# Ascend-Research/HeadPoseEstimation-WHENet

Measured on NVIDIA H100. Metric: head-crops/sec @224x224 bf16, higher is better.
Workload: dtype bf16

## Files before the change

### headposeestimation-whenet_b200/csrc/kernels_dwse.cuh

```cuda
#pragma once
#include <cuda.h>

#include "kernels_fused.cuh"

namespace whenet {
namespace fused {

struct alignas(64) DwSeParams {
    CUtensorMap tmE;
    CUtensorMap tmW;
    CUtensorMap tmX;
    CUtensorMap tmWx;
    const float* b_exp;
    const float* b_dw;
    int* tflag;
    void* out;
    float* partial;
    const float *w_se1t, *b_se1, *w_se2, *b_se2;
    float* gate;
    int Cse;
    float inv_hw;
    int se_tail;
    int scale_out;
    int C, pad;
    int n_chunks, chunks_per_cta;
    int N;
    int tiles_x, Ho_img;
};

template <int KS, int S, int HIN>
struct DwSeGeom {
    static constexpr int HO = (HIN + S - 1) / S;
    static constexpr int R = 7;
    static constexpr int SPR = HO / R;
    static constexpr int NSTRIPS = HO * SPR;
    static constexpr int PW = (HO - 1) * S + KS;
    static constexpr int NCOL = (R - 1) * S + KS;
};

template <int KS, int S, int HIN, int CC>
struct DwSeThreads { static constexpr int value = ((DwSeGeom<KS, S, HIN>::NSTRIPS * (CC / 4)) + 31) / 32 * 32; };

template <int KS, int S, int HIN, int CC>
constexpr size_t dwse_smem(int C, int Cse) {
    using G = DwSeGeom<KS, S, HIN>;
    return (size_t)2 * ((G::PW * G::PW * CC * 2 + 127) / 128 * 128)
           + (size_t)2 * ((CC * 4 + KS * KS * CC * 2 + 127) / 128 * 128)
           + (size_t)2 * G::NSTRIPS * CC * 4
           + (size_t)(C + Cse + 32) * 4 + 256;
}

template <typename T, int KS, int S, int HIN, int CC>
__device__ __forceinline__ void dw_strip(uint32_t erow, uint32_t cst, int cv, T* dst, int C, uint32_t red) {
    using G = DwSeGeom<KS, S, HIN>;
    constexpr int PITCH = CC * 2;
    const float4 bq = lds_f4(cst + (uint32_t)cv * 16);
    const uint32_t cst_h = cst + (uint32_t)(CC * 4 + cv * 8);
    __half2 hacc[G::R][2];
#pragma unroll
    for (int r = 0; r < G::R; ++r) { hacc[r][0] = __float2half2_rn(0.f); hacc[r][1] = __float2half2_rn(0.f); }
#pragma unroll
    for (int ky = 0; ky < KS; ++ky) {
        __half2 wr[KS][2];
#pragma unroll
        for (int kx = 0; kx < KS; ++kx) {
            uint32_t w0, w1;
            lds64(cst_h + (uint32_t)((ky * KS + kx) * CC) * 2, w0, w1);
            wr[kx][0] = *reinterpret_cast<__half2*>(&w0); wr[kx][1] = *reinterpret_cast<__half2*>(&w1);
        }
#pragma unroll
        for (int col = 0; col < G::NCOL; ++col) {
            uint32_t a, b;
            lds64(erow + (uint32_t)(col * PITCH), a, b);
            const __half2 x01 = *reinterpret_cast<__half2*>(&a), x23 = *reinterpret_cast<__half2*>(&b);
#pragma unroll
            for (int r = 0; r < G::R; ++r) {
                const int kx = col - r * S;
                if (kx >= 0 && kx < KS) {
                    hacc[r][0] = __hfma2(x01, wr[kx][0], hacc[r][0]);
                    hacc[r][1] = __hfma2(x23, wr[kx][1], hacc[r][1]);
                }
            }
        }
        erow += G::PW * PITCH;
    }
    const float2 sc = make_float2(kDwScale, kDwScale);
    float sum[4] = {0.f, 0.f, 0.f, 0.f};
#pragma unroll
    for (int r = 0; r < G::R; ++r) {
        float2 a0 = make_float2(bq.x, bq.y), a1 = make_float2(bq.z, bq.w);
        ffma2(a0, __half22float2(hacc[r][0]), sc);
        ffma2(a1, __half22float2(hacc[r][1]), sc);
        a0.x = swish_from_half(a0.x); a0.y = swish_from_half(a0.y);
        a1.x = swish_from_half(a1.x); a1.y = swish_from_half(a1.y);
        sum[0] += a0.x; sum[1] += a0.y; sum[2] += a1.x; sum[3] += a1.y;
        uint2 o;
        o.x = pack2<T>(a0.x, a0.y);
        o.y = pack2<T>(a1.x, a1.y);
        *reinterpret_cast<uint2*>(dst + (long long)r * C) = o;
    }
    asm volatile("st.shared.v4.f32 [%0], {%1,%2,%3,%4};" ::"r"(red), "f"(sum[0]), "f"(sum[1]), "f"(sum[2]), "f"(sum[3]) : "memory");
}

template <int NSTRIPS, int CC>
__device__ __forceinline__ void squeeze_sums(uint32_t red, float* dst, float* means, float inv_hw, int lane) {
    for (int cc = lane; cc < CC; cc += 32) {
        const uint32_t r0 = red + (uint32_t)(cc * 4);
        float s4[4] = {0.f, 0.f, 0.f, 0.f};
#pragma unroll
        for (int y = 0; y < NSTRIPS; ++y) {
            float t;
            asm volatile("ld.shared.f32 %0, [%1];" : "=f"(t) : "r"(r0 + (uint32_t)(y * CC * 4)));
            s4[y & 3] += t;
        }
        const float tot = (s4[0] + s4[1]) + (s4[2] + s4[3]);
        dst[cc] = tot;
        if (means) means[cc] = tot * inv_hw;
    }
}

template <typename T, int NT, int HO>
__device__ __forceinline__ void se_tail_gate(const DwSeParams& p, int n, T* out_n, float* sM) {
    const int C = p.C;
    se_gate_fc<NT>(sM, sM + C, p.w_se1t, p.b_se1, p.w_se2, p.b_se2, p.gate + (long long)n * C, C, p.Cse, sM);
    __syncthreads();
    if (p.scale_out) {
        const int cv8 = C >> 3, total = HO * HO * cv8;
        const float inv_cv8 = 1.0f / (float)cv8;
        for (int v = threadIdx.x; v < total; v += NT) {
            const int c8 = (v - div_small(v, inv_cv8) * cv8) * 8;
            uint4* ptr = reinterpret_cast<uint4*>(out_n) + v;
            *ptr = tc::scale8s<T>(__ldcg(ptr), tc::smem_u32(sM + c8));
        }
    }
}

template <typename T, int KS, int S, int HIN, int CC, bool SPATIAL = false>
__global__ void __launch_bounds__((DwSeThreads<KS, S, HIN, CC>::value)) dwse_kernel(const __grid_constant__ DwSeParams p) {
    using G = DwSeGeom<KS, S, HIN>;
    constexpr int NT = DwSeThreads<KS, S, HIN, CC>::value;
    constexpr int NW = NT / 32;
    constexpr int CV = CC / 4;
    constexpr int PITCH = CC * 2;
    constexpr int TILE_TX = G::PW * G::PW * PITCH;
    constexpr int TILE_BYTES = (TILE_TX + 127) / 128 * 128;
    constexpr int CST_TX = CC * 4 + KS * KS * CC * 2;
    constexpr int CST_BYTES = (CST_TX + 127) / 128 * 128;
    constexpr int RED_BYTES = G::NSTRIPS * CC * 4;
    extern __shared__ __align__(128) uint8_t smem_dw[];
    __shared__ __align__(8) uint64_t bars[4];
    __shared__ int s_abort_mem;
    volatile int* s_abort = &s_abort_mem;
    const uint32_t s0 = (tc::smem_u32(smem_dw) + 127u) & ~127u;
    const uint32_t sT = s0, sC = sT + 2 * TILE_BYTES, sR = sC + 2 * CST_BYTES;
    float* const sM = reinterpret_cast<float*>(smem_dw + (sR + 2 * RED_BYTES - tc::smem_u32(smem_dw)));
    const uint32_t b_full = tc::smem_u32(&bars[0]), b_empty = tc::smem_u32(&bars[2]);

    const int tid = threadIdx.x, warp = tid >> 5, lane = tid & 31;
    const int n = blockIdx.x;
    const int C = p.C;
    const int ch_begin = blockIdx.y * p.chunks_per_cta;
    const int ch_end = min(p.n_chunks, ch_begin + p.chunks_per_cta);
    const int Ho_img = SPATIAL ? p.Ho_img : G::HO;
    T* const out_n = reinterpret_cast<T*>(p.out) + (long long)n * Ho_img * Ho_img * C;

    if (tid == 0) {
        tc::mbar_init(&bars[0], 1); tc::mbar_init(&bars[1], 1);
        tc::mbar_init(&bars[2], NW); tc::mbar_init(&bars[3], NW);
        s_abort_mem = 0;
        asm volatile("fence.mbarrier_init.release.cluster;" ::: "memory");
        asm volatile("prefetch.tensormap [%0];" ::"l"(&p.tmE) : "memory");
        asm volatile("prefetch.tensormap [%0];" ::"l"(&p.tmW) : "memory");
    }
    __syncthreads();

    auto issue = [&](int ch, int buf) {
        const int cbase = SPATIAL ? 0 : ch * CC;
        const uint32_t bar = b_full + 8 * buf;
        tc::mbar::arrive_expect_tx(bar, (uint32_t)(TILE_TX + CST_TX));
        if (SPATIAL) {
            const int ty = ch / p.tiles_x, tx = ch - ty * p.tiles_x;
            tc::mbar::tma_4d(sT + buf * TILE_BYTES, &p.tmE, 0, tx * G::HO * S - p.pad, ty * G::HO * S - p.pad, n, bar);
        } else
            tc::mbar::tma_4d(sT + buf * TILE_BYTES, &p.tmE, cbase, -p.pad, -p.pad, n, bar);
        tc::mbar::tma_2d(sC + buf * CST_BYTES + CC * 4, &p.tmW, cbase, 0, bar);
        asm volatile("cp.async.bulk.shared::cluster.global.mbarrier::complete_tx::bytes [%0], [%1], %2, [%3];"
                     ::"r"(sC + buf * CST_BYTES), "l"(p.b_dw + cbase), "r"((uint32_t)(CC * 4)), "r"(bar) : "memory");
    };

    const int strip = tid / CV, cv = tid - strip * CV;
    const bool active = strip < G::NSTRIPS;
    const int oy = strip / G::SPR, ox0 = (strip - oy * G::SPR) * G::R;
    const uint32_t win = (uint32_t)(((oy * S) * G::PW + ox0 * S) * PITCH + cv * 8);

    if (tid == 0) {
        issue(ch_begin, 0);
        if (ch_begin + 1 < ch_end) issue(ch_begin + 1, 1);
    }

    for (int ch = ch_begin; ch < ch_end; ++ch) {
        const int it = ch - ch_begin, buf = it & 1;
        const uint32_t par = (uint32_t)(it >> 1) & 1u;
        tc::mbar::wait(b_full + 8 * buf, par, s_abort, p.tflag);
        if (active && !*s_abort) {
            T* dst;
            if (SPATIAL) {
                const int ty = ch / p.tiles_x, tx = ch - ty * p.tiles_x;
                dst = out_n + ((long long)(ty * G::HO + oy) * Ho_img + tx * G::HO + ox0) * C + cv * 4;
            } else
                dst = out_n + ((long long)oy * G::HO + ox0) * C + ch * CC + cv * 4;
            dw_strip<T, KS, S, HIN, CC>(sT + buf * TILE_BYTES + win, sC + buf * CST_BYTES, cv, dst, C,
                                        sR + (uint32_t)(buf * RED_BYTES + (strip * CC + cv * 4) * 4));
        }
        tc::mbar::arrive_warp(b_empty + 8 * buf);
        if (warp == 0) {
            tc::mbar::wait(b_empty + 8 * buf, par, s_abort, p.tflag);
            if (SPATIAL) squeeze_sums<G::NSTRIPS, CC>(sR + buf * RED_BYTES, p.partial + ((long long)n * p.n_chunks + ch) * C, nullptr, 0.f, lane);
            else squeeze_sums<G::NSTRIPS, CC>(sR + buf * RED_BYTES, p.partial + (long long)n * C + ch * CC, p.se_tail ? sM + ch * CC : nullptr, p.inv_hw, lane);
            __syncwarp();
            if (lane == 0 && ch + 2 < ch_end) issue(ch + 2, buf);
        }
    }
    __syncthreads();
    if (!SPATIAL && p.se_tail) se_tail_gate<T, NT, G::HO>(p, n, out_n, sM);
}

template <int KS, int S, int HIN, int CC, int CIN>
struct DwSeX {
    using G = DwSeGeom<KS, S, HIN>;
    static constexpr int NT = 256;
    static constexpr int NKB = (CIN + 63) / 64;
    static constexpr int KSTEPS = (CIN + 15) / 16;
    static constexpr int PIX = HIN * HIN;
    static constexpr int HALVES = (PIX + 63) / 64;
    static constexpr int XROWS = (PIX + 7) / 8 * 8;
    static_assert(HALVES == 4 || HALVES == 1, "14x14 or 7x7 maps");
    static constexpr int HPW = HALVES == 4 ? 2 : 1;
    static constexpr int NWG = HALVES == 4 ? CC : CC / 2;
    static_assert(NWG % 16 == 0 && NWG <= 128, "wgmma width");
    static_assert(G::NSTRIPS * (CC / 4) <= NT, "one depthwise strip per thread");
    static constexpr uint32_t X_KB = XROWS * 128, X_BYTES = NKB * X_KB;
    static constexpr uint32_t W_KB = CC * 128, W_BYTES = NKB * W_KB;
    static constexpr uint32_t TILE_BYTES = (G::PW * G::PW * CC * 2 + 127) / 128 * 128;
    static constexpr uint32_t CST_TX = CC * 4 + KS * KS * CC * 2;
    static constexpr uint32_t CST_BYTES = (CST_TX + 127) / 128 * 128;
    static constexpr uint32_t RED_BYTES = G::NSTRIPS * CC * 4;
    static constexpr uint32_t OFF_W = X_BYTES, OFF_T = OFF_W + 2 * W_BYTES, OFF_C = OFF_T + 2 * TILE_BYTES;
    static constexpr uint32_t OFF_R = OFF_C + 2 * CST_BYTES, OFF_M = OFF_R + 2 * RED_BYTES;
    static_assert((X_KB | W_KB | OFF_W | OFF_T) % 1024 == 0, "SWIZZLE_128B operands sit on 1024-byte boundaries");
    static constexpr size_t smem(int C, int Cse) { return (size_t)OFF_M + (size_t)(C + Cse + 32) * 4 + 1024; }
    static constexpr int CTAS_PER_SM = 2 * ((size_t)OFF_M + 4096 + 1024 + 1024) <= 228 * 1024 ? 2 : 1;
};

template <int KS, int S, int HIN, int CC, int CIN>
__global__ void __launch_bounds__(256, (DwSeX<KS, S, HIN, CC, CIN>::CTAS_PER_SM)) dwse_x_kernel(const __grid_constant__ DwSeParams p) {
    using X = DwSeX<KS, S, HIN, CC, CIN>;
    using G = typename X::G;
    using T = __nv_bfloat16;
    constexpr int NT = X::NT;
    constexpr int CV = CC / 4;
    extern __shared__ uint8_t smem_dwx[];
    __shared__ __align__(8) uint64_t bars[5];
    __shared__ int s_abort_mem;
    volatile int* s_abort = &s_abort_mem;
    const uint32_t s0 = (tc::smem_u32(smem_dwx) + 1023u) & ~1023u;
    const uint32_t sX = s0, sW = s0 + X::OFF_W, sT = s0 + X::OFF_T, sC = s0 + X::OFF_C, sR = s0 + X::OFF_R;
    float* const sM = reinterpret_cast<float*>(smem_dwx + (s0 + X::OFF_M - tc::smem_u32(smem_dwx)));
    const uint32_t b_x = tc::smem_u32(&bars[0]), b_w = b_x + 8, b_c = b_x + 24;

    const int tid = threadIdx.x, warp = tid >> 5, lane = tid & 31;
    const int wg = tid >> 7, wq = warp & 3;
    const int n = blockIdx.x;
    const int C = p.C, n_chunks = p.n_chunks;
    T* const out_n = reinterpret_cast<T*>(p.out) + (long long)n * G::HO * G::HO * C;

    if (tid == 0) {
        for (int i = 0; i < 5; ++i) tc::mbar_init(&bars[i], 1);
        s_abort_mem = 0;
        asm volatile("fence.mbarrier_init.release.cluster;" ::: "memory");
        asm volatile("prefetch.tensormap [%0];" ::"l"(&p.tmX) : "memory");
        asm volatile("prefetch.tensormap [%0];" ::"l"(&p.tmWx) : "memory");
        asm volatile("prefetch.tensormap [%0];" ::"l"(&p.tmW) : "memory");
    }
    for (uint32_t o = (uint32_t)tid * 16; o < 2 * X::TILE_BYTES; o += NT * 16) sts128(sT + o, make_uint4(0, 0, 0, 0));
    __syncthreads();

    auto issue_w = [&](int j) {
        const uint32_t bar = b_w + 8 * (j & 1);
        tc::mbar::arrive_expect_tx(bar, X::W_BYTES);
        for (int kb = 0; kb < X::NKB; ++kb) tc::mbar::tma_2d(sW + (j & 1) * X::W_BYTES + kb * X::W_KB, &p.tmWx, kb * 64, j * CC, bar);
    };
    auto issue_c = [&](int j) {
        const uint32_t bar = b_c + 8 * (j & 1), dst = sC + (j & 1) * X::CST_BYTES;
        tc::mbar::arrive_expect_tx(bar, X::CST_TX);
        tc::mbar::tma_2d(dst + CC * 4, &p.tmW, j * CC, 0, bar);
        asm volatile("cp.async.bulk.shared::cluster.global.mbarrier::complete_tx::bytes [%0], [%1], %2, [%3];"
                     ::"r"(dst), "l"(p.b_dw + j * CC), "r"((uint32_t)(CC * 4)), "r"(bar) : "memory");
    };
    if (tid == 0) {
        tc::mbar::arrive_expect_tx(b_x, X::X_BYTES);
        for (int kb = 0; kb < X::NKB; ++kb) tc::mbar::tma_2d(sX + kb * X::X_KB, &p.tmX, kb * 64, n * X::PIX, b_x);
        issue_w(0); issue_c(0);
        if (n_chunks > 1) { issue_w(1); issue_c(1); }
    }

    float acc[X::HPW][X::NWG / 2];
    auto mma = [&](int j) {
        tc::mbar::wait(b_x, 0, s_abort, p.tflag);
        tc::mbar::wait(b_w + 8 * (j & 1), (uint32_t)(j >> 1) & 1u, s_abort, p.tflag);
        const uint32_t wb = sW + (j & 1) * X::W_BYTES;
#pragma unroll
        for (int h = 0; h < X::HPW; ++h) {
            if constexpr (X::HALVES == 4) tc::wg_mma_m64<true, X::NWG>(acc[h], sX + (uint32_t)(wg * X::HPW + h) * 64 * 128, X::X_KB, wb, X::W_KB, X::KSTEPS);
            else tc::wg_mma_m64<true, X::NWG>(acc[h], sX, X::X_KB, wb + (uint32_t)wg * X::NWG * 128, X::W_KB, X::KSTEPS);
        }
    };
    auto epilogue = [&](int j) {
        const uint32_t tile = sT + (j & 1) * X::TILE_BYTES;
        const int c0 = X::HALVES == 4 ? 0 : wg * X::NWG;
        float2 bias[X::NWG / 8];
#pragma unroll
        for (int i = 0; i < X::NWG / 8; ++i) {
            const float* b = p.b_exp + j * CC + c0 + 8 * i + 2 * (lane & 3);
            bias[i] = make_float2(0.5f * __ldg(b), 0.5f * __ldg(b + 1));
        }
#pragma unroll
        for (int h = 0; h < X::HPW; ++h)
#pragma unroll
            for (int e = 0; e < 2; ++e) {
                const int pix = 64 * (X::HALVES == 4 ? wg * X::HPW + h : 0) + 16 * wq + (lane >> 2) + 8 * e;
                if (pix >= X::PIX) continue;
                const int y = pix / HIN, x = pix - y * HIN;
                const uint32_t prow = tile + (uint32_t)(((y + p.pad) * G::PW + x + p.pad) * CC + c0) * 2;
#pragma unroll
                for (int i = 0; i < X::NWG / 8; ++i) {
                    const int c = 8 * i + 2 * (lane & 3);
                    const float o0 = swish_from_half(fmaf(acc[h][4 * i + 2 * e], 0.5f, bias[i].x));
                    const float o1 = swish_from_half(fmaf(acc[h][4 * i + 2 * e + 1], 0.5f, bias[i].y));
                    asm volatile("st.shared.b32 [%0], %1;" ::"r"(prow + (uint32_t)c * 2), "r"(pack2<__half>(o0, o1)) : "memory");
                }
            }
    };

    const int strip = tid / CV, cv = tid - strip * CV;
    const bool active = strip < G::NSTRIPS;
    const int oy = strip / G::SPR, ox0 = (strip - oy * G::SPR) * G::R;
    const uint32_t win = (uint32_t)(((oy * S) * G::PW + ox0 * S) * CC * 2 + cv * 8);

    auto depthwise = [&](int j) {
        tc::mbar::wait(b_c + 8 * (j & 1), (uint32_t)(j >> 1) & 1u, s_abort, p.tflag);
        if (active && !*s_abort)
            dw_strip<T, KS, S, HIN, CC>(sT + (j & 1) * X::TILE_BYTES + win, sC + (j & 1) * X::CST_BYTES, cv,
                                        out_n + ((long long)oy * G::HO + ox0) * C + j * CC + cv * 4, C,
                                        sR + (uint32_t)((j & 1) * X::RED_BYTES + (strip * CC + cv * 4) * 4));
    };
    auto close = [&](int j) {
        if (warp == 0)
            squeeze_sums<G::NSTRIPS, CC>(sR + (j & 1) * X::RED_BYTES, p.partial + (long long)n * C + j * CC,
                                         p.se_tail ? sM + j * CC : nullptr, p.inv_hw, lane);
        if (tid == 0) {
            if (j + 3 < n_chunks) issue_w(j + 3);
            if (j + 2 < n_chunks) issue_c(j + 2);
        }
    };

    mma(0);
    tc::wg_wait<0>();
    epilogue(0);
    __syncthreads();
    if (tid == 0 && 2 < n_chunks) issue_w(2);
    for (int j = 0; j + 1 < n_chunks; ++j) {
        mma(j + 1);
        depthwise(j);
        tc::wg_wait<0>();
        epilogue(j + 1);
        __syncthreads();
        close(j);
    }
    depthwise(n_chunks - 1);
    __syncthreads();
    close(n_chunks - 1);
    __syncthreads();
    if (p.se_tail) se_tail_gate<T, NT, G::HO>(p, n, out_n, sM);
}

inline int dwse_chunk(int k, int s, int hin, int C) {
    if (hin == 14 && s == 1 && (k == 3 || k == 5) && C % 32 == 0) return 32;
    if (hin == 14 && s == 2 && k == 5 && C % 96 == 0) return 96;
    if (hin == 7 && s == 1 && (k == 3 || k == 5) && C % 128 == 0) return 128;
    return 0;
}

template <typename T>
int launch_dwse(cudaStream_t stream, DwSeParams p, int k, int s, int hin, int n_crops, int split) {
    const int CCr = dwse_chunk(k, s, hin, p.C);
    if (!CCr) return 1;
    p.N = n_crops;
    p.n_chunks = p.C / CCr;
    if (split < 1) split = 1;
    if (split > p.n_chunks) split = p.n_chunks;
    p.chunks_per_cta = (p.n_chunks + split - 1) / split;
    const int gy = (p.n_chunks + p.chunks_per_cta - 1) / p.chunks_per_cta;
    if (gy > 1) { p.se_tail = 0; p.scale_out = 0; }
#define DWSE(KS, S, HIN, CC)                                                                                              \
    do {                                                                                                                  \
        auto kfn = dwse_kernel<T, KS, S, HIN, CC>;                                                                        \
        const size_t smem = dwse_smem<KS, S, HIN, CC>(p.C, p.Cse);                                                        \
        if (cudaFuncSetAttribute(kfn, cudaFuncAttributeMaxDynamicSharedMemorySize, (int)smem) != cudaSuccess) return -1;  \
        kfn<<<dim3(n_crops, gy), DwSeThreads<KS, S, HIN, CC>::value, smem, stream>>>(p);                                    \
        return 0;                                                                                                         \
    } while (0)
    if (hin == 14 && s == 1 && k == 3) DWSE(3, 1, 14, 32);
    if (hin == 14 && s == 1 && k == 5) DWSE(5, 1, 14, 32);
    if (hin == 14 && s == 2 && k == 5) DWSE(5, 2, 14, 96);
    if (hin == 7 && s == 1 && k == 5) DWSE(5, 1, 7, 128);
    if (hin == 7 && s == 1 && k == 3) DWSE(3, 1, 7, 128);
#undef DWSE
    return 1;
}


template <typename T>
int launch_dwse_x(cudaStream_t stream, DwSeParams p, int k, int s, int hin, int cin, int n_crops) {
    static_assert(std::is_same<T, __nv_bfloat16>::value, "the on-chip expand runs the bf16 wgmma");
    const int CCr = dwse_chunk(k, s, hin, p.C);
    if (!CCr) return 1;
    p.N = n_crops;
    p.n_chunks = p.C / CCr;
    p.chunks_per_cta = p.n_chunks;
#define DWSEX(KS, S, HIN, CC, CIN)                                                                                        \
    do {                                                                                                                  \
        auto kfn = dwse_x_kernel<KS, S, HIN, CC, CIN>;                                                                    \
        const size_t smem = DwSeX<KS, S, HIN, CC, CIN>::smem(p.C, p.Cse);                                                 \
        if (cudaFuncSetAttribute(kfn, cudaFuncAttributeMaxDynamicSharedMemorySize, (int)smem) != cudaSuccess) return -1;  \
        kfn<<<n_crops, DwSeX<KS, S, HIN, CC, CIN>::NT, smem, stream>>>(p);                                                \
        return 0;                                                                                                         \
    } while (0)
    if (CCr == 32 && hin == 14 && s == 1 && k == 3 && cin == 80) DWSEX(3, 1, 14, 32, 80);
    if (CCr == 32 && hin == 14 && s == 1 && k == 5 && cin == 80) DWSEX(5, 1, 14, 32, 80);
    if (CCr == 32 && hin == 14 && s == 1 && k == 5 && cin == 112) DWSEX(5, 1, 14, 32, 112);
    if (CCr == 96 && hin == 14 && s == 2 && k == 5 && cin == 112) DWSEX(5, 2, 14, 96, 112);
    if (CCr == 128 && hin == 7 && s == 1 && k == 5 && cin == 192) DWSEX(5, 1, 7, 128, 192);
    if (CCr == 128 && hin == 7 && s == 1 && k == 3 && cin == 192) DWSEX(3, 1, 7, 128, 192);
#undef DWSEX
    return 1;
}

template <typename T>
int launch_dwse_spatial(cudaStream_t stream, DwSeParams p, int H, int n_crops, int split) {
    if (p.C != 32 || H % 14) return 1;
    p.N = n_crops;
    p.tiles_x = H / 14; p.Ho_img = H;
    p.n_chunks = p.tiles_x * p.tiles_x;
    if (split < 1) split = 1;
    if (split > p.n_chunks) split = p.n_chunks;
    p.chunks_per_cta = (p.n_chunks + split - 1) / split;
    const int gy = (p.n_chunks + p.chunks_per_cta - 1) / p.chunks_per_cta;
    p.se_tail = 0; p.scale_out = 0;
    auto kfn = dwse_kernel<T, 3, 1, 14, 32, true>;
    const size_t smem = dwse_smem<3, 1, 14, 32>(0, 0);
    if (cudaFuncSetAttribute(kfn, cudaFuncAttributeMaxDynamicSharedMemorySize, (int)smem) != cudaSuccess) return -1;
    kfn<<<dim3(n_crops, gy), DwSeThreads<3, 1, 14, 32>::value, smem, stream>>>(p);
    return 0;
}

}
}
```

Baseline: 87840.

## Process two crops per CTA in fused expand+depthwise kernel for 14x14 k5 layers

Templates the fused expand/depthwise/SE kernel on a crops-per-CTA count and enables two crops per CTA for the 14x14 stride-1 5x5 layers with 80 and 112 input channels. Each loaded weight chunk (expand weights and depthwise taps) is reused across both crops, and the depthwise inner loop reuses the register-held taps for two strips. This cuts weight traffic and per-CTA fixed overhead. In exchange it doubles per-CTA shared memory and register accumulators, which may reduce occupancy, and it halves the grid size.

New measurement: 87790 (median of 6 runs). Within noise of the previous version (-0.1%).

```diff
diff --git a/headposeestimation-whenet_b200/csrc/kernels_dwse.cuh b/headposeestimation-whenet_b200/csrc/kernels_dwse.cuh
--- a/headposeestimation-whenet_b200/csrc/kernels_dwse.cuh
+++ b/headposeestimation-whenet_b200/csrc/kernels_dwse.cuh
@@ -50,15 +50,21 @@
            + (size_t)(C + Cse + 32) * 4 + 256;
 }
 
-template <typename T, int KS, int S, int HIN, int CC>
-__device__ __forceinline__ void dw_strip(uint32_t erow, uint32_t cst, int cv, T* dst, int C, uint32_t red) {
+template <typename T, int KS, int S, int HIN, int CC, int NS>
+__device__ __forceinline__ void dw_strip(const uint32_t (&erow)[NS], uint32_t cst, int cv, T* const (&dst)[NS], int C,
+                                         const uint32_t (&red)[NS], int nstore) {
     using G = DwSeGeom<KS, S, HIN>;
     constexpr int PITCH = CC * 2;
     const float4 bq = lds_f4(cst + (uint32_t)cv * 16);
     const uint32_t cst_h = cst + (uint32_t)(CC * 4 + cv * 8);
-    __half2 hacc[G::R][2];
-#pragma unroll
-    for (int r = 0; r < G::R; ++r) { hacc[r][0] = __float2half2_rn(0.f); hacc[r][1] = __float2half2_rn(0.f); }
+    __half2 hacc[NS][G::R][2];
+    uint32_t e[NS];
+#pragma unroll
+    for (int s = 0; s < NS; ++s) {
+        e[s] = erow[s];
+#pragma unroll
+        for (int r = 0; r < G::R; ++r) { hacc[s][r][0] = __float2half2_rn(0.f); hacc[s][r][1] = __float2half2_rn(0.f); }
+    }
 #pragma unroll
     for (int ky = 0; ky < KS; ++ky) {
         __half2 wr[KS][2];
@@ -70,36 +76,43 @@
         }
 #pragma unroll
         for (int col = 0; col < G::NCOL; ++col) {
-            uint32_t a, b;
-            lds64(erow + (uint32_t)(col * PITCH), a, b);
-            const __half2 x01 = *reinterpret_cast<__half2*>(&a), x23 = *reinterpret_cast<__half2*>(&b);
-#pragma unroll
-            for (int r = 0; r < G::R; ++r) {
-                const int kx = col - r * S;
-                if (kx >= 0 && kx < KS) {
-                    hacc[r][0] = __hfma2(x01, wr[kx][0], hacc[r][0]);
-                    hacc[r][1] = __hfma2(x23, wr[kx][1], hacc[r][1]);
+#pragma unroll
+            for (int s = 0; s < NS; ++s) {
+                uint32_t a, b;
+                lds64(e[s] + (uint32_t)(col * PITCH), a, b);
+                const __half2 x01 = *reinterpret_cast<__half2*>(&a), x23 = *reinterpret_cast<__half2*>(&b);
+#pragma unroll
+                for (int r = 0; r < G::R; ++r) {
+                    const int kx = col - r * S;
+                    if (kx >= 0 && kx < KS) {
+                        hacc[s][r][0] = __hfma2(x01, wr[kx][0], hacc[s][r][0]);
+                        hacc[s][r][1] = __hfma2(x23, wr[kx][1], hacc[s][r][1]);
+                    }
                 }
             }
         }
-        erow += G::PW * PITCH;
+#pragma unroll
+        for (int s = 0; s < NS; ++s) e[s] += G::PW * PITCH;
     }
     const float2 sc = make_float2(kDwScale, kDwScale);
-    float sum[4] = {0.f, 0.f, 0.f, 0.f};
-#pragma unroll
-    for (int r = 0; r < G::R; ++r) {
-        float2 a0 = make_float2(bq.x, bq.y), a1 = make_float2(bq.z, bq.w);
-        ffma2(a0, __half22float2(hacc[r][0]), sc);
-        ffma2(a1, __half22float2(hacc[r][1]), sc);
-        a0.x = swish_from_half(a0.x); a0.y = swish_from_half(a0.y);
-        a1.x = swish_from_half(a1.x); a1.y = swish_from_half(a1.y);
-        sum[0] += a0.x; sum[1] += a0.y; sum[2] += a1.x; sum[3] += a1.y;
-        uint2 o;
-        o.x = pack2<T>(a0.x, a0.y);
-        o.y = pack2<T>(a1.x, a1.y);
-        *reinterpret_cast<uint2*>(dst + (long long)r * C) = o;
-    }
-    asm volatile("st.shared.v4.f32 [%0], {%1,%2,%3,%4};" ::"r"(red), "f"(sum[0]), "f"(sum[1]), "f"(sum[2]), "f"(sum[3]) : "memory");
+#pragma unroll
+    for (int s = 0; s < NS; ++s) {
+        float sum[4] = {0.f, 0.f, 0.f, 0.f};
+#pragma unroll
+        for (int r = 0; r < G::R; ++r) {
+            float2 a0 = make_float2(bq.x, bq.y), a1 = make_float2(bq.z, bq.w);
+            ffma2(a0, __half22float2(hacc[s][r][0]), sc);
+            ffma2(a1, __half22float2(hacc[s][r][1]), sc);
+            a0.x = swish_from_half(a0.x); a0.y = swish_from_half(a0.y);
+            a1.x = swish_from_half(a1.x); a1.y = swish_from_half(a1.y);
+            sum[0] += a0.x; sum[1] += a0.y; sum[2] += a1.x; sum[3] += a1.y;
+            uint2 o;
+            o.x = pack2<T>(a0.x, a0.y);
+            o.y = pack2<T>(a1.x, a1.y);
+            if (s < nstore) *reinterpret_cast<uint2*>(dst[s] + (long long)r * C) = o;
+        }
+        asm volatile("st.shared.v4.f32 [%0], {%1,%2,%3,%4};" ::"r"(red[s]), "f"(sum[0]), "f"(sum[1]), "f"(sum[2]), "f"(sum[3]) : "memory");
+    }
 }
 
 template <int NSTRIPS, int CC>
@@ -209,8 +222,8 @@
                 dst = out_n + ((long long)(ty * G::HO + oy) * Ho_img + tx * G::HO + ox0) * C + cv * 4;
             } else
                 dst = out_n + ((long long)oy * G::HO + ox0) * C + ch * CC + cv * 4;
-            dw_strip<T, KS, S, HIN, CC>(sT + buf * TILE_BYTES + win, sC + buf * CST_BYTES, cv, dst, C,
-                                        sR + (uint32_t)(buf * RED_BYTES + (strip * CC + cv * 4) * 4));
+            dw_strip<T, KS, S, HIN, CC, 1>({sT + buf * TILE_BYTES + win}, sC + buf * CST_BYTES, cv, {dst}, C,
+                                           {sR + (uint32_t)(buf * RED_BYTES + (strip * CC + cv * 4) * 4)}, 1);
         }
         tc::mbar::arrive_warp(b_empty + 8 * buf);
         if (warp == 0) {
@@ -225,10 +238,11 @@
     if (!SPATIAL && p.se_tail) se_tail_gate<T, NT, G::HO>(p, n, out_n, sM);
 }
 
-template <int KS, int S, int HIN, int CC, int CIN>
+template <int KS, int S, int HIN, int CC, int CIN, int NC>
 struct DwSeX {
     using G = DwSeGeom<KS, S, HIN>;
     static constexpr int NT = 256;
+    static_assert(NC == 1 || NC == 2, "one or two crops per CTA");
     static constexpr int NKB = (CIN + 63) / 64;
     static constexpr int KSTEPS = (CIN + 15) / 16;
     static constexpr int PIX = HIN * HIN;
@@ -245,20 +259,22 @@
     static constexpr uint32_t CST_TX = CC * 4 + KS * KS * CC * 2;
     static constexpr uint32_t CST_BYTES = (CST_TX + 127) / 128 * 128;
     static constexpr uint32_t RED_BYTES = G::NSTRIPS * CC * 4;
-    static constexpr uint32_t OFF_W = X_BYTES, OFF_T = OFF_W + 2 * W_BYTES, OFF_C = OFF_T + 2 * TILE_BYTES;
-    static constexpr uint32_t OFF_R = OFF_C + 2 * CST_BYTES, OFF_M = OFF_R + 2 * RED_BYTES;
+    static constexpr uint32_t OFF_W = NC * X_BYTES, OFF_T = OFF_W + 2 * W_BYTES, OFF_C = OFF_T + 2 * NC * TILE_BYTES;
+    static constexpr uint32_t OFF_R = OFF_C + 2 * CST_BYTES, OFF_M = OFF_R + 2 * NC * RED_BYTES;
     static_assert((X_KB | W_KB | OFF_W | OFF_T) % 1024 == 0, "SWIZZLE_128B operands sit on 1024-byte boundaries");
-    static constexpr size_t smem(int C, int Cse) { return (size_t)OFF_M + (size_t)(C + Cse + 32) * 4 + 1024; }
-    static constexpr int CTAS_PER_SM = 2 * ((size_t)OFF_M + 4096 + 1024 + 1024) <= 228 * 1024 ? 2 : 1;
+    __host__ __device__ static constexpr int m_floats(int C, int Cse) { return (C + Cse + 32 + 3) / 4 * 4; }
+    static constexpr size_t smem(int C, int Cse) { return (size_t)OFF_M + (size_t)NC * m_floats(C, Cse) * 4 + 1024; }
+    static constexpr int CTAS_PER_SM = 2 * ((size_t)OFF_M + NC * 4096 + 1024 + 1024) <= 228 * 1024 ? 2 : 1;
 };
 
-template <int KS, int S, int HIN, int CC, int CIN>
-__global__ void __launch_bounds__(256, (DwSeX<KS, S, HIN, CC, CIN>::CTAS_PER_SM)) dwse_x_kernel(const __grid_constant__ DwSeParams p) {
-    using X = DwSeX<KS, S, HIN, CC, CIN>;
+template <int KS, int S, int HIN, int CC, int CIN, int NC>
+__global__ void __launch_bounds__(256, (DwSeX<KS, S, HIN, CC, CIN, NC>::CTAS_PER_SM)) dwse_x_kernel(const __grid_constant__ DwSeParams p) {
+    using X = DwSeX<KS, S, HIN, CC, CIN, NC>;
     using G = typename X::G;
     using T = __nv_bfloat16;
     constexpr int NT = X::NT;
     constexpr int CV = CC / 4;
+    constexpr long long CROP_OUT = (long long)G::HO * G::HO;
     extern __shared__ uint8_t smem_dwx[];
     __shared__ __align__(8) uint64_t bars[5];
     __shared__ int s_abort_mem;
@@ -270,9 +286,11 @@
 
     const int tid = threadIdx.x, warp = tid >> 5, lane = tid & 31;
     const int wg = tid >> 7, wq = warp & 3;
-    const int n = blockIdx.x;
+    const int n0 = blockIdx.x * NC;
+    const int nc = NC == 1 ? 1 : min(NC, p.N - n0);
     const int C = p.C, n_chunks = p.n_chunks;
-    T* const out_n = reinterpret_cast<T*>(p.out) + (long long)n * G::HO * G::HO * C;
+    const int mfl = X::m_floats(C, p.Cse);
+    T* const out0 = reinterpret_cast<T*>(p.out) + (long long)n0 * CROP_OUT * C;
 
     if (tid == 0) {
         for (int i = 0; i < 5; ++i) tc::mbar_init(&bars[i], 1);
@@ -282,7 +300,7 @@
         asm volatile("prefetch.tensormap [%0];" ::"l"(&p.tmWx) : "memory");
         asm volatile("prefetch.tensormap [%0];" ::"l"(&p.tmW) : "memory");
     }
-    for (uint32_t o = (uint32_t)tid * 16; o < 2 * X::TILE_BYTES; o += NT * 16) sts128(sT + o, make_uint4(0, 0, 0, 0));
+    for (uint32_t o = (uint32_t)tid * 16; o < 2 * NC * X::TILE_BYTES; o += NT * 16) sts128(sT + o, make_uint4(0, 0, 0, 0));
     __syncthreads();
 
     auto issue_w = [&](int j) {
@@ -298,25 +316,28 @@
                      ::"r"(dst), "l"(p.b_dw + j * CC), "r"((uint32_t)(CC * 4)), "r"(bar) : "memory");
     };
     if (tid == 0) {
-        tc::mbar::arrive_expect_tx(b_x, X::X_BYTES);
-        for (int kb = 0; kb < X::NKB; ++kb) tc::mbar::tma_2d(sX + kb * X::X_KB, &p.tmX, kb * 64, n * X::PIX, b_x);
+        tc::mbar::arrive_expect_tx(b_x, (uint32_t)nc * X::X_BYTES);
+        for (int c = 0; c < nc; ++c)
+            for (int kb = 0; kb < X::NKB; ++kb) tc::mbar::tma_2d(sX + c * X::X_BYTES + kb * X::X_KB, &p.tmX, kb * 64, (n0 + c) * X::PIX, b_x);
         issue_w(0); issue_c(0);
         if (n_chunks > 1) { issue_w(1); issue_c(1); }
     }
 
-    float acc[X::HPW][X::NWG / 2];
+    float acc[NC][X::HPW][X::NWG / 2];
     auto mma = [&](int j) {
         tc::mbar::wait(b_x, 0, s_abort, p.tflag);
         tc::mbar::wait(b_w + 8 * (j & 1), (uint32_t)(j >> 1) & 1u, s_abort, p.tflag);
         const uint32_t wb = sW + (j & 1) * X::W_BYTES;
 #pragma unroll
-        for (int h = 0; h < X::HPW; ++h) {
-            if constexpr (X::HALVES == 4) tc::wg_mma_m64<true, X::NWG>(acc[h], sX + (uint32_t)(wg * X::HPW + h) * 64 * 128, X::X_KB, wb, X::W_KB, X::KSTEPS);
-            else tc::wg_mma_m64<true, X::NWG>(acc[h], sX, X::X_KB, wb + (uint32_t)wg * X::NWG * 128, X::W_KB, X::KSTEPS);
-        }
+        for (int c = 0; c < NC; ++c)
+#pragma unroll
+            for (int h = 0; h < X::HPW; ++h) {
+                const uint32_t xc = sX + (uint32_t)c * X::X_BYTES;
+                if constexpr (X::HALVES == 4) tc::wg_mma_m64<true, X::NWG>(acc[c][h], xc + (uint32_t)(wg * X::HPW + h) * 64 * 128, X::X_KB, wb, X::W_KB, X::KSTEPS);
+                else tc::wg_mma_m64<true, X::NWG>(acc[c][h], xc, X::X_KB, wb + (uint32_t)wg * X::NWG * 128, X::W_KB, X::KSTEPS);
+            }
     };
     auto epilogue = [&](int j) {
-        const uint32_t tile = sT + (j & 1) * X::TILE_BYTES;
         const int c0 = X::HALVES == 4 ? 0 : wg * X::NWG;
         float2 bias[X::NWG / 8];
 #pragma unroll
@@ -325,21 +346,25 @@
             bias[i] = make_float2(0.5f * __ldg(b), 0.5f * __ldg(b + 1));
         }
 #pragma unroll
-        for (int h = 0; h < X::HPW; ++h)
-#pragma unroll
-            for (int e = 0; e < 2; ++e) {
-                const int pix = 64 * (X::HALVES == 4 ? wg * X::HPW + h : 0) + 16 * wq + (lane >> 2) + 8 * e;
-                if (pix >= X::PIX) continue;
-                const int y = pix / HIN, x = pix - y * HIN;
-                const uint32_t prow = tile + (uint32_t)(((y + p.pad) * G::PW + x + p.pad) * CC + c0) * 2;
-#pragma unroll
-                for (int i = 0; i < X::NWG / 8; ++i) {
-                    const int c = 8 * i + 2 * (lane & 3);
-                    const float o0 = swish_from_half(fmaf(acc[h][4 * i + 2 * e], 0.5f, bias[i].x));
-                    const float o1 = swish_from_half(fmaf(acc[h][4 * i + 2 * e + 1], 0.5f, bias[i].y));
-                    asm volatile("st.shared.b32 [%0], %1;" ::"r"(prow + (uint32_t)c * 2), "r"(pack2<__half>(o0, o1)) : "memory");
+        for (int c = 0; c < NC; ++c) {
+            const uint32_t tile = sT + (uint32_t)((j & 1) * NC + c) * X::TILE_BYTES;
+#pragma unroll
+            for (int h = 0; h < X::HPW; ++h)
+#pragma unroll
+                for (int e = 0; e < 2; ++e) {
+                    const int pix = 64 * (X::HALVES == 4 ? wg * X::HPW + h : 0) + 16 * wq + (lane >> 2) + 8 * e;
+                    if (pix >= X::PIX) continue;
+                    const int y = pix / HIN, x = pix - y * HIN;
+                    const uint32_t prow = tile + (uint32_t)(((y + p.pad) * G::PW + x + p.pad) * CC + c0) * 2;
+#pragma unroll
+                    for (int i = 0; i < X::NWG / 8; ++i) {
+                        const int cc = 8 * i + 2 * (lane & 3);
+                        const float o0 = swish_from_half(fmaf(acc[c][h][4 * i + 2 * e], 0.5f, bias[i].x));
+                        const float o1 = swish_from_half(fmaf(acc[c][h][4 * i + 2 * e + 1], 0.5f, bias[i].y));
+                        asm volatile("st.shared.b32 [%0], %1;" ::"r"(prow + (uint32_t)cc * 2), "r"(pack2<__half>(o0, o1)) : "memory");
+                    }
                 }
-            }
+        }
     };
 
     const int strip = tid / CV, cv = tid - strip * CV;
@@ -349,15 +374,22 @@
 
     auto depthwise = [&](int j) {
         tc::mbar::wait(b_c + 8 * (j & 1), (uint32_t)(j >> 1) & 1u, s_abort, p.tflag);
-        if (active && !*s_abort)
-            dw_strip<T, KS, S, HIN, CC>(sT + (j & 1) * X::TILE_BYTES + win, sC + (j & 1) * X::CST_BYTES, cv,
-                                        out_n + ((long long)oy * G::HO + ox0) * C + j * CC + cv * 4, C,
-                                        sR + (uint32_t)((j & 1) * X::RED_BYTES + (strip * CC + cv * 4) * 4));
+        if (active && !*s_abort) {
+            uint32_t erow[NC], red[NC];
+            T* dst[NC];
+#pragma unroll
+            for (int c = 0; c < NC; ++c) {
+                erow[c] = sT + (uint32_t)((j & 1) * NC + c) * X::TILE_BYTES + win;
+                dst[c] = out0 + c * CROP_OUT * C + ((long long)oy * G::HO + ox0) * C + j * CC + cv * 4;
+                red[c] = sR + (uint32_t)(((j & 1) * NC + c) * X::RED_BYTES + (strip * CC + cv * 4) * 4);
+            }
+            dw_strip<T, KS, S, HIN, CC, NC>(erow, sC + (j & 1) * X::CST_BYTES, cv, dst, C, red, nc);
+        }
     };
     auto close = [&](int j) {
-        if (warp == 0)
-            squeeze_sums<G::NSTRIPS, CC>(sR + (j & 1) * X::RED_BYTES, p.partial + (long long)n * C + j * CC,
-                                         p.se_tail ? sM + j * CC : nullptr, p.inv_hw, lane);
+        if (warp < nc)
+            squeeze_sums<G::NSTRIPS, CC>(sR + (uint32_t)((j & 1) * NC + warp) * X::RED_BYTES, p.partial + (long long)(n0 + warp) * C + j * CC,
+                                         p.se_tail ? sM + warp * mfl + j * CC : nullptr, p.inv_hw, lane);
         if (tid == 0) {
             if (j + 3 < n_chunks) issue_w(j + 3);
             if (j + 2 < n_chunks) issue_c(j + 2);
@@ -381,7 +413,8 @@
     __syncthreads();
     close(n_chunks - 1);
     __syncthreads();
-    if (p.se_tail) se_tail_gate<T, NT, G::HO>(p, n, out_n, sM);
+    if (p.se_tail)
+        for (int c = 0; c < nc; ++c) se_tail_gate<T, NT, G::HO>(p, n0 + c, out0 + c * CROP_OUT * C, sM + c * mfl);
 }
 
 inline int dwse_chunk(int k, int s, int hin, int C) {
@@ -428,20 +461,20 @@
     p.N = n_crops;
     p.n_chunks = p.C / CCr;
     p.chunks_per_cta = p.n_chunks;
-#define DWSEX(KS, S, HIN, CC, CIN)                                                                                        \
+#define DWSEX(KS, S, HIN, CC, CIN, NC)                                                                                    \
     do {                                                                                                                  \
-        auto kfn = dwse_x_kernel<KS, S, HIN, CC, CIN>;                                                                    \
-        const size_t smem = DwSeX<KS, S, HIN, CC, CIN>::smem(p.C, p.Cse);                                                 \
+        auto kfn = dwse_x_kernel<KS, S, HIN, CC, CIN, NC>;                                                                \
+        const size_t smem = DwSeX<KS, S, HIN, CC, CIN, NC>::smem(p.C, p.Cse);                                             \
         if (cudaFuncSetAttribute(kfn, cudaFuncAttributeMaxDynamicSharedMemorySize, (int)smem) != cudaSuccess) return -1;  \
-        kfn<<<n_crops, DwSeX<KS, S, HIN, CC, CIN>::NT, smem, stream>>>(p);                                                \
+        kfn<<<(n_crops + NC - 1) / NC, DwSeX<KS, S, HIN, CC, CIN, NC>::NT, smem, stream>>>(p);                            \
         return 0;                                                                                                         \
     } while (0)
-    if (CCr == 32 && hin == 14 && s == 1 && k == 3 && cin == 80) DWSEX(3, 1, 14, 32, 80);
-    if (CCr == 32 && hin == 14 && s == 1 && k == 5 && cin == 80) DWSEX(5, 1, 14, 32, 80);
-    if (CCr == 32 && hin == 14 && s == 1 && k == 5 && cin == 112) DWSEX(5, 1, 14, 32, 112);
-    if (CCr == 96 && hin == 14 && s == 2 && k == 5 && cin == 112) DWSEX(5, 2, 14, 96, 112);
-    if (CCr == 128 && hin == 7 && s == 1 && k == 5 && cin == 192) DWSEX(5, 1, 7, 128, 192);
-    if (CCr == 128 && hin == 7 && s == 1 && k == 3 && cin == 192) DWSEX(3, 1, 7, 128, 192);
+    if (CCr == 32 && hin == 14 && s == 1 && k == 3 && cin == 80) DWSEX(3, 1, 14, 32, 80, 1);
+    if (CCr == 32 && hin == 14 && s == 1 && k == 5 && cin == 80) DWSEX(5, 1, 14, 32, 80, 2);
+    if (CCr == 32 && hin == 14 && s == 1 && k == 5 && cin == 112) DWSEX(5, 1, 14, 32, 112, 2);
+    if (CCr == 96 && hin == 14 && s == 2 && k == 5 && cin == 112) DWSEX(5, 2, 14, 96, 112, 1);
+    if (CCr == 128 && hin == 7 && s == 1 && k == 5 && cin == 192) DWSEX(5, 1, 7, 128, 192, 1);
+    if (CCr == 128 && hin == 7 && s == 1 && k == 3 && cin == 192) DWSEX(3, 1, 7, 128, 192, 1);
 #undef DWSEX
     return 1;
 }
```
